# DarianNwankwo/Rollout-Bayesian-Optimization

Measured on AMD Instinct MI355X. Metric: rollout trajectories/sec (MC samples × restarts) at horizon h=3, n=64 GP, higher is better.
Workload: dtype f64

## Files before the change

rollout-bayesian-optimization_amd/csrc/mrbo_rollout.hip:

```cpp
#include <utility>

#include "mrbo_device.h"
#include "bcast_asm.h"
#include "mrbo_lane_tables.h"

#ifndef MRBO_WAVES_PER_SIMD
#define MRBO_WAVES_PER_SIMD 2
#endif
#define MRBO_FNS_CAT_(a, b) a##b
#define MRBO_FNS_CAT(a, b) MRBO_FNS_CAT_(a, b)
#define MRBO_FNS MRBO_FNS_CAT(fmax, MRBO_FMAX)
#ifndef MRBO_WAVES_PER_SIMD_GL
#define MRBO_WAVES_PER_SIMD_GL 1
#endif

namespace mrbo {
inline namespace MRBO_FNS {

constexpr double PAD_FAR = 1e100;

template <int D, int RPL, int HW = 1>
struct Lay {
  static constexpr int D1 = D + 1;
  static constexpr int BS = (D1 + 1) & ~1;
  static constexpr int NR = RPL * WAVE;
  static constexpr int LANES = WAVE / HW;
  static constexpr int NRL = RPL * LANES;
  static constexpr bool SQ = (RPL == 1);
  static constexpr bool BC = (RPL <= 2);
  static constexpr int FR0 = 0;
  static constexpr int BROWS = FR0 + FMAX;
  static constexpr int NG = D1 * (D1 + 1) / 2;
  static constexpr int NH = D * (D + 1) / 2;
  static constexpr int R_VAL = 0;
  static constexpr int R_G = 8;
  static constexpr int NGC = (NG - 1 + 15) / 16;
  static constexpr int R_MF = R_G + 16 * NGC;
  static constexpr int NMF = D * (1 + FMAX);
  static constexpr int NMFC = (NMF + 15) / 16;
  static constexpr int NPAIR = D * D + 2 * D;
  static constexpr int NPC = (NPAIR + 15) / 16;
  static constexpr int NHC = (NH + 1 + 15) / 16;
  static constexpr int REDN_A = R_MF + 16 * NMFC;
  static constexpr int REDN_B = 16 * (NPC > NHC ? NPC : NHC);
  static constexpr int REDN = ((REDN_A > REDN_B ? REDN_A : REDN_B) + 1) & ~1;
  static constexpr int U_X = 0;
  static constexpr int DE = (D + 1) & ~1;
  static constexpr int U_XB = U_X + (DE > 8 ? DE : 8);
  static constexpr int U_XF = U_XB + (DE > 8 ? DE : 8);
  static constexpr int U_YF = U_XF + FMAX * D;
  static constexpr int U_GF = U_YF + FMAX;
  static constexpr int U_DINV = U_GF + FMAX * D;
  static constexpr int U_CF = U_DINV + FMAX * FMAX;
  static constexpr int U_FMIN = U_CF + (FMAX + 1) * FMAX;
  static constexpr int U_SC = U_FMIN + FMAX + 1;
  static constexpr int U_GMU = U_SC + 20;
  static constexpr int U_GSIG = U_GMU + D;
  static constexpr int U_GAL = U_GSIG + D;
  static constexpr int U_MIX = U_GAL + D;
  static constexpr int U_G = U_MIX + D;
  static constexpr int U_H = U_G + D1 * D1;
  static constexpr int U_YFV = U_H + D * D;
  static constexpr int U_WF = U_YFV + FMAX * D1;
  static constexpr int U_PF = U_WF + FMAX;
  static constexpr int U_GMU0 = U_PF + FMAX * D;
  static constexpr int U_XBAR = U_GMU0 + D;
  static constexpr int U_ACC = U_XBAR + FMAX * D;
  static constexpr int U_YBAR = U_ACC + FMAX * D;
  static constexpr int U_DX = U_YBAR + FMAX + 1;
  static constexpr int U_NX = U_DX + D;
  static constexpr int U_NG = U_NX + D;
  static constexpr int U_NP = U_NG + D;
  static constexpr int U_LB = U_NP + D;
  static constexpr int U_UB = U_LB + D;
  static constexpr int U_HF = U_UB + D;
  static constexpr int U_STAMP = U_HF + FMAX * (D + 2);
  static constexpr int U_KC = U_STAMP + NSTAMP_SLOTS;
  static constexpr bool LTAB = (RPL == 1);
  static constexpr int U_TAB = ((U_KC + 15) + 1) & ~1;
  static constexpr int U_SIZE = LTAB ? ((U_TAB + LaneTables<D, FMAX>::DOUBLES + 1) & ~1) : U_TAB;
  static constexpr int G12 = 3 * NRL;
  static constexpr int EC = SQ ? (2 * FMAX + 1) * NRL : 0;
// ... 308 lines not shown
      for (int q = 0; q < 8; ++q) v[q] = fill(16 * ch + q);
      hw_reduce<HW, 8>(v, red + 16 * ch, lane);
    } else {
      double v[16];
#pragma unroll
      for (int q = 0; q < 16; ++q) v[q] = fill(16 * ch + q);
      hw_reduce<HW, 16>(v, red + 16 * ch, lane);
    }
  }
}

template <int K>
__device__ __forceinline__ void gl_bcast_product_k(double (&acc)[K], const double (&v)[K], const double* lb, int nrows) {
#pragma unroll
  for (int p = 0; p < 2; ++p) {
    if (16 * p >= nrows) break;
    double l[4][8];
#pragma unroll
    for (int u = 0; u < 8; ++u) {
      l[0][u] = lb[(16 * p + u) * WAVE];
      l[1][u] = lb[(16 * p + 8 + u) * WAVE];
      l[2][u] = lb[(16 * (p + 2) + u) * WAVE];
      l[3][u] = lb[(16 * (p + 2) + 8 + u) * WAVE];
    }
    double bp[K], bp2[K];
#pragma unroll
    for (int c = 0; c < K; ++c) {
      if (p == 0) row_blocks<0>(v[c], bp[c], bp2[c]);
      else row_blocks<1>(v[c], bp[c], bp2[c]);
    }
    BcastRegAsm<K, 0>::run(acc, bp, l[0]);
    BcastRegAsm<K, 8>::run(acc, bp, l[1]);
    if (16 * (p + 2) < nrows) {
      BcastRegAsm<K, 0>::run(acc, bp2, l[2]);
      BcastRegAsm<K, 8>::run(acc, bp2, l[3]);
    }
  }
}

template <int K>
__device__ __forceinline__ void gl_bcast_product(double (&acc)[K], const double (&v)[K], const double* lb, int nrows) {
  if constexpr (K > 9) {
    gl_bcast_product<8>(head8(acc), head8(v), lb, nrows);
    gl_bcast_product<K - 8>(tail8(acc), tail8(v), lb, nrows);
  } else {
    gl_bcast_product_k<K>(acc, v, lb, nrows);
  }
}

template <int K, int LD, int NLB>
__device__ __forceinline__ void gl_block(double (&acc)[K], const double (&v)[K], const double* Lg, const double* LinvL,
                                         int b, bool fwd, int lane, int nrows) {
  const int li = NLB > 0 ? gl_lds_slot(b) : -1;
  if (li >= 0) {
    const double* sq = LinvL + (long long)li * WAVE * LD;
    if (fwd) bcast_product<K, LD, 1, false>(acc, v, sq + lane, nrows);
    else bcast_product<K, 1, 1, false>(acc, v, sq + lane * LD, nrows);
  } else {
    gl_bcast_product<K>(acc, v, Lg + (long long)b * WAVE * WAVE + lane, nrows);
  }
}

template <int D, int RPL, int HW>
__device__ __forceinline__ bool newton_pg_ok(WaveCtx<D, RPL, HW>& W, const KParams& kp);

struct NewtonState {
  double f, ft, dec, t;
  int it, ls;
  int st;
  bool trial;
  int why;
};
enum { NT_STOP = 0,
       NT_BACKTRACK = 1,
       NT_CONTINUE = 2 };
template <int D, int RPL, int HW>
__device__ __forceinline__ int newton_after_value(WaveCtx<D, RPL, HW>& W, const KParams& kp, int S, NewtonState& ns);

constexpr int EV_RT = -1;

template <int D, int RPL, int HW, int MODE = EV_RT>
__device__ __forceinline__ int evaluate(WaveCtx<D, RPL, HW>& W, const KParams& kp, int S, int mode_rt,
                                        LaneRes<D, RPL, HW>& lr, int kst = 0, bool back_after = false,
                                        NewtonState* nt = nullptr) {
  using Ly = Lay<D, RPL, HW>;
  constexpr int D1 = Ly::D1, BS = Ly::BS, NR = Ly::NR;
  constexpr bool FUSABLE = Ly::SQ && HW == 1;
  static_assert(MODE == EV_RT || (MODE >= EV_VALUE && MODE <= EV_GSTART), "evaluate: MODE");
  const int mode = MODE == EV_RT ? mode_rt : MODE;
  int lane = W.lane;
  asm volatile("" : "+v"(lane));
  const int nf = S + 1;
  double* U = W.U;
  double* B = W.B;
  double* red = W.red;
  const unsigned* tab = reinterpret_cast<const unsigned*>(U + Ly::U_TAB);
  const bool all_cols = (mode != EV_VALUE);
  const bool do_val = (mode != EV_GRADC);
  STAMP(W, 8);

  double x[D];
#pragma unroll
  for (int a = 0; a < D; ++a) x[a] = U[Ly::U_X + a];

  double Ev[RPL][FMAX];
#pragma unroll
  for (int s = 0; s < RPL; ++s) {
    lr.cb[s] = W.C[(long long)(S + 1) * Ly::NRL + lane + WAVE * s];
#pragma unroll
    for (int r = 0; r < FMAX; ++r) Ev[s][r] = W.E[(long long)r * Ly::NRL + lane + WAVE * s];
#pragma unroll
    for (int r = 0; r < FMAX; ++r) Ev[s][r] = (r < nf) ? Ev[s][r] : 0.0;
  }

  const int N = W.N;
  double acc[RPL][D1];
  if (mode != EV_BACK) {
  double Bown[RPL][D1];
  double rf[D], psif = 0.0, g1f = 0.0, g2f = 0.0;
  const bool rows_kept = (mode == EV_GRADC);
#pragma unroll
  for (int s = 0; s < RPL; ++s) {
    double r[D], rho2 = 0.0;
#pragma unroll
    for (int a = 0; a < D; ++a) { r[a] = x[a] - W.X0[s][a]; rho2 = fma(r[a], r[a], rho2); }
    if (rows_kept) {
      const double g1 = W.G12[3 * (lane + WAVE * s)];
      const bool v = W.rowv(kp, s);
      Bown[s][0] = 0.0;
#pragma unroll
      for (int a = 0; a < D; ++a) Bown[s][1 + a] = v ? g1 * r[a] : 0.0;
      continue;
    }
    double psi, g1, g2;
    if constexpr (RPL == 1) {
      const int fl = lane < nf ? lane : 0;
      double rho2f = 0.0;
#pragma unroll
      for (int a = 0; a < D; ++a) { rf[a] = x[a] - U[Ly::U_XF + fl * D + a]; rho2f = fma(rf[a], rf[a], rho2f); }
      rad_eval2<MODE != EV_RT>(W.rad, rho2, rho2f, psi, g1, g2, psif, g1f, g2f);
    } else {
      rad_eval(W.rad, rho2, psi, g1, g2);
    }
    const bool v = W.rowv(kp, s);
    Bown[s][0] = v ? psi : 0.0;
#pragma unroll
    for (int a = 0; a < D; ++a) Bown[s][1 + a] = v ? g1 * r[a] : 0.0;
    W.G12[3 * (lane + WAVE * s)] = g1;
    W.G12[3 * (lane + WAVE * s) + 1] = g2;
  }
  if (lane < nf && !rows_kept) {
    double r[D], psi, g1, g2;
    if constexpr (RPL == 1) {
#pragma unroll
      for (int a = 0; a < D; ++a) r[a] = rf[a];
      psi = psif;
      g1 = g1f;
      g2 = g2f;
    } else {
      double rho2 = 0.0;
#pragma unroll
      for (int a = 0; a < D; ++a) { r[a] = x[a] - U[Ly::U_XF + lane * D + a]; rho2 = fma(r[a], r[a], rho2); }
      rad_eval(W.rad, rho2, psi, g1, g2);
    }
    double* row = B + (Ly::FR0 + lane) * BS;
    row[0] = psi;
#pragma unroll
    for (int a = 0; a < D; ++a) row[1 + a] = g1 * r[a];
    {
      double* hf = U + Ly::U_HF + lane * (D + 2);
#pragma unroll
      for (int a = 0; a < D; ++a) hf[a] = r[a];
      hf[D] = g1;
      hf[D + 1] = g2;
    }
  }
  wave_sync();
  STAMP(W, 0);

#pragma unroll
  for (int s = 0; s < RPL; ++s)
#pragma unroll
    for (int c = 0; c < D1; ++c) acc[s][c] = 0.0;
  if constexpr (Ly::BC) {
    auto nrows = [&](int t) { const int n = N - WAVE * t; return n < WAVE ? n : WAVE; };
    const bool fold = Ly::SQ && HW == 1 && N > 48;
#ifdef MRBO_BC_DIAG_FOLD
    constexpr bool DFOLD = !Ly::SQ && HW == 1;
#else
    constexpr bool DFOLD = false;
#endif
    if (mode == EV_VALUE) {
#pragma unroll
      for (int s = 0; s < RPL; ++s) {
        double a1[1] = {0.0};
#pragma unroll
        for (int t = 0; t <= s; ++t) {
          const double v1[1] = {Bown[t][0]};
          if (fold) bcast_fold_fwd<1>(a1, v1, W.Linv, lane);
          else if (DFOLD && s == t && nrows(t) > 48) bcast_fold_fwd<1>(a1, v1, W.Linv + Ly::blk(s, t) * Ly::BLK, lane);
          else bcast_product<1, Ly::LD, HW>(a1, v1, W.Linv + Ly::blk(s, t) * Ly::BLK + lane, nrows(t));
        }
        acc[s][0] = a1[0];
      }
    } else if (mode == EV_GSTART) {
      if constexpr (Ly::SQ) acc[0][0] = W.YTAB[(long long)kst * NR + lane];
    } else if (mode == EV_GRADC) {
#pragma unroll
      for (int s = 0; s < RPL; ++s) {
        double ag[D];
#pragma unroll
        for (int a = 0; a < D; ++a) ag[a] = 0.0;
#pragma unroll
        for (int t = 0; t <= s; ++t) {
          double vg[D];
#pragma unroll
          for (int a = 0; a < D; ++a) vg[a] = Bown[t][1 + a];
          if (fold) bcast_fold_fwd<D>(ag, vg, W.Linv, lane);
          else if (DFOLD && s == t && nrows(t) > 48) bcast_fold_fwd<D>(ag, vg, W.Linv + Ly::blk(s, t) * Ly::BLK, lane);
          else bcast_product<D, Ly::LD, HW>(ag, vg, W.Linv + Ly::blk(s, t) * Ly::BLK + lane, nrows(t));
        }
#pragma unroll
        for (int a = 0; a < D; ++a) acc[s][1 + a] = ag[a];
        acc[s][0] = W.G12[3 * (lane + WAVE * s) + 2];
      }
    } else {
#pragma unroll
      for (int s = 0; s < RPL; ++s)
#pragma unroll
        for (int t = 0; t <= s; ++t) {
          if (fold) bcast_fold_fwd<D1>(acc[s], Bown[t], W.Linv, lane);
          else if (DFOLD && s == t && nrows(t) > 48) bcast_fold_fwd<D1>(acc[s], Bown[t], W.Linv + Ly::blk(s, t) * Ly::BLK, lane);
          else bcast_product<D1, Ly::LD, HW>(acc[s], Bown[t], W.Linv + Ly::blk(s, t) * Ly::BLK + lane, nrows(t));
        }
    }
  } else {
    auto nrows = [&](int t) { const int n = N - WAVE * t; return n < WAVE ? n : WAVE; };
    const double* L0 = W.Linv + lane;
    if (mode == EV_VALUE) {
#pragma unroll
      for (int s = 0; s < RPL; ++s) {
        double a1[1] = {0.0};
#pragma unroll
        for (int t = 0; t <= s; ++t) {
          const double v1[1] = {Bown[t][0]};
          gl_block<1, Ly::LD, Ly::NLB>(a1, v1, W.Linv, W.LinvL, Ly::blk(s, t), true, lane, nrows(t));
        }
        acc[s][0] = a1[0];
      }
    } else if (mode == EV_GRADC) {
#pragma unroll
      for (int s = 0; s < RPL; ++s) {
// ... 94 lines not shown
#pragma unroll
    for (int r = 0; r < FMAX; ++r) {
      if (r < nf) {
        g00_v = fma(yf[r], yf[r], g00_v);
        mu_v = fma(U[Ly::U_CF + (S + 1) * FMAX + r], bf[r], mu_v);
      }
    }
    if (lane < FMAX) {
      double mine = 0.0;
#pragma unroll
      for (int r = 0; r < FMAX; ++r) mine = (lane == r) ? yf[r] : mine;
      if (lane < nf) U[Ly::U_YFV + lane * D1] = mine;
    }
    if (lane == 0) {
      U[Ly::U_G] = g00_v;
      U[Ly::U_SC + SC_MU] = mu_v;
    }
  }
  if (all_cols) {
  {
    const int ncol = D;
    for (int t = lane; t < (FMAX * D <= Ly::LANES ? Ly::LANES : FMAX * D); t += Ly::LANES) {
      if (t >= nf * ncol) break;
      int r = t / ncol, c = 1 + t % ncol;
      if constexpr (Ly::LTAB) {
        const unsigned tw = tab[t];
        r = lane_field(tw, LaneWord::R, LaneWord::W3);
        c = lane_field(tw, LaneWord::C, LaneWord::W5);
      }
      double y = red[Ly::R_MF + D + r * D + (c - 1)];
      for (int q = 0; q <= r; ++q) y = fma(U[Ly::U_DINV + r * FMAX + q], B[(Ly::FR0 + q) * BS + c], y);
      U[Ly::U_YFV + r * D1 + c] = y;
      if constexpr (FMAX * D <= Ly::LANES) break;
    }
  }
  wave_sync();
  {
    auto gram_entry = [&](int t) {
      int a = 0, b;
      if constexpr (Ly::LTAB) {
        const unsigned tw = tab[t];
        a = lane_field(tw, LaneWord::GA, LaneWord::W5);
        b = lane_field(tw, LaneWord::GB, LaneWord::W5);
      } else {
        int rem = t;
#pragma unroll
        for (int aa = 0; aa < D1; ++aa) if (a == aa && rem >= D1 - aa) { rem -= D1 - aa; a = aa + 1; }
        b = a + rem;
      }
      double g = (mode == EV_GSTART) ? W.GTAB[kst * Ly::NG + t] : red[Ly::R_G + t - 1];
      for (int r = 0; r < nf; ++r) g = fma(U[Ly::U_YFV + r * D1 + a], U[Ly::U_YFV + r * D1 + b], g);
      U[Ly::U_G + a * D1 + b] = g;
      U[Ly::U_G + b * D1 + a] = g;
    };
    auto gmu_entry = [&](int c) {
      double mu = red[Ly::R_MF + c - 1];
      for (int r = 0; r < nf; ++r) mu = fma(U[Ly::U_CF + (S + 1) * FMAX + r], B[(Ly::FR0 + r) * BS + c], mu);
      U[Ly::U_GMU + c - 1] = mu;
    };
    if constexpr (HW == 2) {
      static_assert(Ly::NG <= 16 && 16 + D <= 32, "half-wave Gram placement");
      if (lane > 0 && lane < Ly::NG) gram_entry(lane);
      if (lane >= 16 && lane < 16 + D) gmu_entry(lane - 15);
    } else if constexpr (Ly::NG <= 49) {
      if (lane > 0 && lane < Ly::NG) gram_entry(lane);
      if (lane >= 49 && lane < 48 + D1) gmu_entry(lane - 48);
    } else {
      for (int t = lane; t < Ly::NG; t += WAVE)
        if (t > 0) gram_entry(t);
      if (lane >= 1 && lane <= D) gmu_entry(lane);
    }
  }
  wave_sync();
  }
  STAMP(W, 3);

  double isig_f;
  EIp e_f;
  if (do_val) {
  const double mu = mu_v;
  const double var = KCV(PSI0) - g00_v;
  double sig, isig;
  sig_isig(var, sig, isig);
  const double fmin = U[Ly::U_FMIN + S + 1];
  const EIp e = rule_partials(kp.rule, mu, sig, KCV(THETA), fmin, KCV(SIGTOL), isig);
  double alpha = e.g;
  if (kp.cost) {
    double gc[D];
    const double c = cost_eval<D>(kp, x, gc);
    double gmax = 0.0;
#pragma unroll
    for (int a = 0; a < D; ++a) gmax = fmax(gmax, fabs(gc[a]));
    alpha = e.g / c;
    if (lane == 0) {
      U[Ly::U_SC + SC_ARAW] = e.g;
      U[Ly::U_SC + SC_COSTC] = c;
      U[Ly::U_SC + SC_GCMAX] = gmax;
    }
  }
  if (lane == 0) {
    U[Ly::U_SC + SC_SIG] = sig;
    U[Ly::U_SC + SC_ISIG] = isig;
    U[Ly::U_SC + SC_VAR] = var;
    U[Ly::U_SC + SC_ALPHA] = alpha;
    U[Ly::U_SC + SC_GMU] = e.gmu;
    U[Ly::U_SC + SC_GSIG] = e.gsig;
    U[Ly::U_SC + SC_GMUMU] = e.gmumu;
    U[Ly::U_SC + SC_GSIGSIG] = e.gsigsig;
    U[Ly::U_SC + SC_GMUTH] = e.gmuth;
    U[Ly::U_SC + SC_GSIGTH] = e.gsigth;
    U[Ly::U_SC + SC_FMIN] = fmin;
  }
  if (mode == EV_VALUE) {
    wave_sync();
    STAMP(W, 4);
    if constexpr (FUSABLE) {
      if (nt != nullptr) {
        nt->why = newton_after_value<D, RPL, HW>(W, kp, S, *nt);
        if (nt->why != NT_CONTINUE || !kp.newton_fused) return 0;
        if constexpr (MODE != EV_GRADC)
          return EVR_GRAD | evaluate<D, RPL, HW, EV_GRADC>(W, kp, S, EV_GRADC, lr, kst, true);
      }
    }
    return 0;
  }
  isig_f = isig;
  e_f = e;
  } else {
    isig_f = U[Ly::U_SC + SC_ISIG];
    e_f.gmu = U[Ly::U_SC + SC_GMU];
    e_f.gsig = U[Ly::U_SC + SC_GSIG];
    e_f.gmuth = U[Ly::U_SC + SC_GMUTH];
    e_f.gsigth = U[Ly::U_SC + SC_GSIGTH];
  }
  if (lane < D) {
    const double gs = -U[Ly::U_G + (1 + lane) * D1] * isig_f;
    const double gm = U[Ly::U_GMU + lane];
    U[Ly::U_GSIG + lane] = gs;
    double gal = e_f.gmu * gm + e_f.gsig * gs;
    double mix = gm * e_f.gmuth + gs * e_f.gsigth;
    if (kp.cost) {
      double gc[D];
      (void)cost_eval<D>(kp, x, gc);
      const double gca = lane_pick<D>(gc, lane);
      const double c = U[Ly::U_SC + SC_COSTC], araw = U[Ly::U_SC + SC_ARAW];
      gal = gal / c - (araw / (c * c)) * gca;
      mix = mix / c - rule_gth(kp.rule, e_f.gmu, U[Ly::U_SC + SC_SIG]) * gca / (c * c);
    }
    U[Ly::U_GAL + lane] = gal;
    U[Ly::U_MIX + lane] = mix;
  }
  if (mode == EV_GRAD || mode == EV_GRADC || mode == EV_GSTART) {
    wave_sync();
    STAMP(W, 4);
    if (!back_after) return 0;
    if (lane < D) U[Ly::U_NG + lane] = -U[Ly::U_GAL + lane];
    wave_sync();
    if (!newton_pg_ok<D, RPL, HW>(W, kp)) return 0;
    STAMP(W, 12);
  }
  } else {
#pragma unroll
    for (int s = 0; s < RPL; ++s) acc[s][0] = W.G12[3 * (lane + WAVE * s) + 2];
  }
  wave_sync();
  EIp e;
  e.gmu = U[Ly::U_SC + SC_GMU];
  e.gsig = U[Ly::U_SC + SC_GSIG];
  e.gmumu = U[Ly::U_SC + SC_GMUMU];
  e.gsigsig = U[Ly::U_SC + SC_GSIGSIG];

  STAMP(W, 4);
  const bool rich = (mode == EV_RICH);
  {
    double wv[RPL], pv[RPL][D];
#pragma unroll
    for (int s = 0; s < RPL; ++s) {
      wv[s] = 0.0;
#pragma unroll
      for (int a = 0; a < D; ++a) pv[s][a] = 0.0;
    }
    if constexpr (Ly::BC) {
      auto nrows = [&](int t) { const int n = N - WAVE * t; return n < WAVE ? n : WAVE; };
      const bool fold = Ly::SQ && HW == 1 && N > 48;
#ifdef MRBO_BC_DIAG_FOLD
      constexpr bool DFOLD = !Ly::SQ && HW == 1;
#else
      constexpr bool DFOLD = false;
#endif
#pragma unroll
      for (int s = 0; s < RPL; ++s) {
        if (rich) {
          double a7[D1];
#pragma unroll
          for (int c = 0; c < D1; ++c) a7[c] = 0.0;
#pragma unroll
          for (int t = s; t < RPL; ++t) {
            if (fold) bcast_fold_bwd<D1>(a7, acc[t], W.Linv, lane);
            else if (DFOLD && s == t && nrows(t) > 48) bcast_fold_bwd<D1>(a7, acc[t], W.Linv + Ly::blk(t, s) * Ly::BLK, lane);
            else bcast_product<D1, 1, HW>(a7, acc[t], W.Linv + Ly::blk(t, s) * Ly::BLK + lane * Ly::LD, nrows(t));
          }
          wv[s] = a7[0];
#pragma unroll
          for (int a = 0; a < D; ++a) pv[s][a] = a7[1 + a];
        } else {
          double a1[1] = {0.0};
#pragma unroll
          for (int t = s; t < RPL; ++t) {
            const double v1[1] = {acc[t][0]};
            if (fold) bcast_fold_bwd<1>(a1, v1, W.Linv, lane);
            else if (DFOLD && s == t && nrows(t) > 48) bcast_fold_bwd<1>(a1, v1, W.Linv + Ly::blk(t, s) * Ly::BLK, lane);
            else bcast_product<1, 1, HW>(a1, v1, W.Linv + Ly::blk(t, s) * Ly::BLK + lane * Ly::LD, nrows(t));
          }
          wv[s] = a1[0];
        }
      }
    } else {
      auto nrows = [&](int t) { const int n = N - WAVE * t; return n < WAVE ? n : WAVE; };
      const double* LT = W.LinvT + lane;
#pragma unroll
      for (int s = 0; s < RPL; ++s) {
        if (rich) {
          double a7[D1];
#pragma unroll
          for (int c = 0; c < D1; ++c) a7[c] = 0.0;
#pragma unroll
          for (int t = s; t < RPL; ++t)
            gl_block<D1, Ly::LD, Ly::NLB>(a7, acc[t], W.LinvT, W.LinvL, Ly::blk(t, s), false, lane, nrows(t));
          wv[s] = a7[0];
#pragma unroll
          for (int a = 0; a < D; ++a) pv[s][a] = a7[1 + a];
        } else {
          double a1[1] = {0.0};
#pragma unroll
          for (int t = s; t < RPL; ++t) {
            const double v1[1] = {acc[t][0]};
            gl_block<1, Ly::LD, Ly::NLB>(a1, v1, W.LinvT, W.LinvL, Ly::blk(t, s), false, lane, nrows(t));
          }
          wv[s] = a1[0];
        }
      }
    }
#pragma unroll
    for (int s = 0; s < RPL; ++s) {
#pragma unroll
      for (int r = 0; r < FMAX; ++r) {
        if (r >= nf) break;
        const double er = Ev[s][r];
// ... 32 lines not shown
    for (int s = 0; s < RPL; ++s) {
#pragma unroll
      for (int a = 0; a < D; ++a) nv[s][a] = x[a] - W.X0[s][a];
      const double coef = W.rowv(kp, s) ? (e.gmu * lr.cb[s] - gsig_over * lr.w[s]) : 0.0;
      ca[s] = coef * W.G12[3 * (lane + WAVE * s) + 1];
      tb[s] = coef * W.G12[3 * (lane + WAVE * s)];
    }
    wave_sync();
    auto hval = [&](int t) {
      double s_ = 0.0;
      if (t < Ly::NH) {
        int a = 0, rem = t;
#pragma unroll
        for (int aa = 0; aa < D; ++aa) if (a == aa && rem >= D - aa) { rem -= D - aa; a = aa + 1; }
        const int b = a + rem;
#pragma unroll
        for (int s = 0; s < RPL; ++s) s_ = fma(ca[s], nv[s][a] * nv[s][b], s_);
      } else if (t == Ly::NH) {
#pragma unroll
        for (int s = 0; s < RPL; ++s) s_ += tb[s];
      }
      return s_;
    };
    constexpr int HTAIL = (Ly::NH + 1) % 16;
    constexpr int HFULL = (HTAIL > 0 && HTAIL <= 8) ? (Ly::NH + 1) / 16 : Ly::NHC;
#pragma unroll
    for (int ch = 0; ch < HFULL; ++ch) {
      double vv[16];
#pragma unroll
      for (int q = 0; q < 16; ++q) vv[q] = hval(16 * ch + q);
      hw_reduce<HW, 16>(vv, red + 16 * ch, lane);
    }
    if constexpr (HFULL < Ly::NHC) {
      double vv[8];
#pragma unroll
      for (int q = 0; q < 8; ++q) vv[q] = hval(16 * HFULL + q);
      hw_reduce<HW, 8>(vv, red + 16 * HFULL, lane);
    }
  }
  wave_sync();
  STAMP(W, 6);
  for (int he = lane; he < (Ly::NH <= Ly::LANES ? Ly::LANES : Ly::NH); he += Ly::LANES) {
    if (he >= Ly::NH) break;
    int a = 0, b;
    if constexpr (Ly::LTAB) {
      const unsigned tw = tab[he];
      a = lane_field(tw, LaneWord::HA, LaneWord::W5);
      b = lane_field(tw, LaneWord::HB, LaneWord::W5);
    } else {
      int rem = he;
#pragma unroll
      for (int aa = 0; aa < D; ++aa) if (a == aa && rem >= D - aa) { rem -= D - aa; a = aa + 1; }
      b = a + rem;
    }
    const double gma = U[Ly::U_GMU + a], gmb = U[Ly::U_GMU + b];
    const double gsa = U[Ly::U_GSIG + a], gsb = U[Ly::U_GSIG + b];
    const double rdiag = red[Ly::NH];
    double hv = red[he] + ((a == b) ? rdiag : 0.0);
    for (int r = 0; r < nf; ++r) {
      const double* hf = U + Ly::U_HF + r * (D + 2);
      const double coef = e.gmu * U[Ly::U_CF + (S + 1) * FMAX + r] - gsig_over * U[Ly::U_WF + r];
      hv = fma(coef * hf[D + 1], hf[a] * hf[b], hv);
      if (a == b) hv = fma(coef, hf[D], hv);
    }
    hv += e.gmumu * gma * gmb + e.gsigsig * gsa * gsb - gsig_over * (gsa * gsb + U[Ly::U_G + (1 + a) * D1 + 1 + b]);
    if (kp.cost) {
      double gc[D];
      (void)cost_eval<D>(kp, x, gc);
      const double gca = lane_pick<D>(gc, a), gcb = lane_pick<D>(gc, b);
      const double c = U[Ly::U_SC + SC_COSTC], araw = U[Ly::U_SC + SC_ARAW];
      hv = (hv - U[Ly::U_GAL + a] * gcb - gca * U[Ly::U_GAL + b]) / c - (araw / (c * c)) * cost_hess<D>(kp, c, a, b);
    }
    U[Ly::U_H + a * D + b] = hv;
    U[Ly::U_H + b * D + a] = hv;
    if constexpr (Ly::NH <= Ly::LANES) break;
  }
  wave_sync();
  STAMP(W, 7);
  return EVR_BACK;
}

template <int D, int RPL, int HW>
__device__ __forceinline__ int condition(WaveCtx<D, RPL, HW>& W, const KParams& kp, int S, double yv, const double* gy,
                         const LaneRes<D, RPL, HW>& lr) {
  using Ly = Lay<D, RPL, HW>;
  constexpr int NR = Ly::NR;
  double* U = W.U;
  const int lane = W.ln();
  const int nf = S + 1;
  const double g00 = U[Ly::U_G];
  const double mu = U[Ly::U_SC + SC_MU];
  const double l22sq = KCV(PSI0) + KCV(SN2) - g00;
  if (!(l22sq > 0.0)) return 4;
  const double inv = 1.0 / sqrt(l22sq);
  const double gam = (yv - mu) / l22sq;
#pragma unroll
  for (int s = 0; s < RPL; ++s) {
    const int i = lane + WAVE * s;
    W.E[(long long)nf * Ly::NRL + i] = W.rowv(kp, s) ? -lr.w[s] * inv : 0.0;
    W.C[(long long)(S + 2) * Ly::NRL + i] = W.rowv(kp, s) ? (lr.cb[s] - gam * lr.w[s]) : 0.0;
  }
  wave_sync();
  if (lane < nf) {
    const double wq = U[Ly::U_WF + lane];
    U[Ly::U_DINV + nf * FMAX + lane] = -wq * inv;
    U[Ly::U_CF + (S + 2) * FMAX + lane] = U[Ly::U_CF + (S + 1) * FMAX + lane] - gam * wq;
  }
  if (lane == nf) {
    U[Ly::U_DINV + nf * FMAX + nf] = inv;
    U[Ly::U_CF + (S + 2) * FMAX + nf] = gam;
    U[Ly::U_YF + nf] = yv;
    const double fm = U[Ly::U_FMIN + S + 1];
    U[Ly::U_FMIN + S + 2] = (yv < fm) ? yv : fm;
  }
  double gmine = 0.0;
#pragma unroll
  for (int a = 0; a < D; ++a) gmine = (a == lane) ? gy[a] : gmine;
  if (lane < D) {
    U[Ly::U_XF + nf * D + lane] = U[Ly::U_X + lane];
    U[Ly::U_GF + nf * D + lane] = gmine;
  }
  wave_sync();
  return 0;
}

template <int D, int RPL, int HW>
__device__ __forceinline__ int draw_factor(WaveCtx<D, RPL, HW>& W, double (&Lc)[Lay<D, RPL, HW>::NG]) {
  using Ly = Lay<D, RPL, HW>;
  constexpr int D1 = Ly::D1;
  const double* U = W.U;
#define TRI(i, j) ((i) * ((i) + 1) / 2 + (j))
#pragma unroll
  for (int j = 0; j < D1; ++j) {
    const double kjj = (j == 0) ? KCV(PSI0) : -KCV(D2PSI0);
    double sdiag = kjj - U[Ly::U_G + j * D1 + j];
#pragma unroll
    for (int k = 0; k < j; ++k) sdiag -= Lc[TRI(j, k)] * Lc[TRI(j, k)];
    if (!(sdiag > 0.0)) return 2;
    double ljj, ij;
    sqrt_rsqrt(sdiag, ljj, ij);
    Lc[TRI(j, j)] = ljj;
#pragma unroll
    for (int i = j + 1; i < D1; ++i) {
      double t = -U[Ly::U_G + j * D1 + i];
#pragma unroll
      for (int k = 0; k < j; ++k) t -= Lc[TRI(i, k)] * Lc[TRI(j, k)];
      Lc[TRI(i, j)] = t * ij;
    }
  }
#undef TRI
  return 0;
}

template <int D, int RPL, int HW>
__device__ __forceinline__ int draw(WaveCtx<D, RPL, HW>& W, const KParams& kp, const double* z, double& yv, double* gy,
                                    const double* hdr = nullptr) {
  using Ly = Lay<D, RPL, HW>;
  constexpr int D1 = Ly::D1;
  const double* U = W.U;
  double Lc[Ly::NG];
#define TRI(i, j) ((i) * ((i) + 1) / 2 + (j))
  if (hdr) {
    if (hdr[RT_FAIL] != 0.0) return 2;
#pragma unroll
    for (int i = 0; i < Ly::NG; ++i) Lc[i] = hdr[RT_GMU + 2 * D + i];
  } else if (draw_factor<D, RPL, HW>(W, Lc)) {
    return 2;
  }
  double out[D1];
  out[0] = U[Ly::U_SC + SC_MU];
#pragma unroll
  for (int a = 0; a < D; ++a) out[1 + a] = U[Ly::U_GMU + a];
#pragma unroll
  for (int a = 0; a < D1; ++a) {
    double s = 0.0;
#pragma unroll
    for (int k = 0; k <= a; ++k) s += Lc[TRI(a, k)] * z[k];
    out[a] += s;
  }
#undef TRI
  yv = out[0];
#pragma unroll
  for (int a = 0; a < D; ++a) gy[a] = out[1 + a];
  return 0;
}

template <int D>
__device__ __forceinline__ bool chol_packed(double (&A)[D * (D + 1) / 2], double (&idg)[D]) {
#define TRI(i, j) ((i) * ((i) + 1) / 2 + (j))
  bool ok = true;
#pragma unroll
  for (int j = 0; j < D; ++j) {
    double s = A[TRI(j, j)];
#pragma unroll
    for (int k = 0; k < j; ++k) s -= A[TRI(j, k)] * A[TRI(j, k)];
    ok = ok && (s > 0.0);
    if (!ok) return false;
    double ljj;
    sqrt_rsqrt(s, ljj, idg[j]);
    A[TRI(j, j)] = ljj;
#pragma unroll
    for (int i = j + 1; i < D; ++i) {
      double t = A[TRI(i, j)];
#pragma unroll
      for (int k = 0; k < j; ++k) t -= A[TRI(i, k)] * A[TRI(j, k)];
      A[TRI(i, j)] = t * idg[j];
    }
  }
#undef TRI
  return ok;
}

template <int D, int RPL, int HW>
__device__ __forceinline__ bool newton_pg_ok(WaveCtx<D, RPL, HW>& W, const KParams& kp) {
  using Ly = Lay<D, RPL, HW>;
  const double* U = W.U;
  const int lane = W.ln();
  const int a = lane < D ? lane : 0;
  const double xs = U[Ly::U_NX + a], gs = U[Ly::U_NG + a], lb = U[Ly::U_LB + a], ub = U[Ly::U_UB + a];
  const bool act = ((xs <= lb) & (gs > 0.0)) | ((xs >= ub) & (gs < 0.0));
  const bool fr = (lane < D) & !act;
  const unsigned long long fm = hw_ballot<HW>(fr, W.half);
  const unsigned long long big = hw_ballot<HW>(fr & (fabs(gs) > KCV(GTOL)), W.half);
  if (lane == 0) W.U[Ly::U_SC + SC_FREE] = (double)(unsigned)fm;
  return big != 0ull;
}

template <int D, int RPL, int HW, bool ALL_FREE>
__device__ __forceinline__ bool newton_direction_fm(WaveCtx<D, RPL, HW>& W, const KParams& kp, int fm) {
  using Ly = Lay<D, RPL, HW>;
  constexpr int NH = D * (D + 1) / 2;
  double* U = W.U;
  const int lane = W.ln();
  bool fr[D];
  double gs[D];
#pragma unroll
  for (int a = 0; a < D; ++a) {
    fr[a] = ALL_FREE || ((fm >> a) & 1);
    gs[a] = U[Ly::U_NG + a];
  }
  double A0[NH];
#pragma unroll
  for (int i = 0; i < D; ++i)
#pragma unroll
    for (int j = 0; j <= i; ++j) {
      const double h = U[Ly::U_H + i * D + j];
      A0[i * (i + 1) / 2 + j] = (fr[i] && fr[j]) ? -h : ((i == j) ? 1.0 : 0.0);
    }
  double tau = 0.0, hmax = 0.0;
#pragma unroll
  for (int i = 0; i < D; ++i) {
    double off = 0.0;
#pragma unroll
// ... 322 lines not shown
  for (int q = threadIdx.x; q < NR * ns; q += blockDim.x) {
    const int i = q / ns, k = q - (q / ns) * ns;
    double v = 0.0;
    if (i < kp.N) {
      double rho2 = 0.0;
#pragma unroll
      for (int a = 0; a < D; ++a) {
        const double r = clampd(xs[k * D + a], kp.lbs[a], kp.ubs[a]) - kp.X0[(long long)a * NR + i];
        rho2 = fma(r, r, rho2);
      }
      double g1, g2;
      rad_eval(rad, rho2, v, g1, g2);
    }
    kxb[q] = v;
  }
  __syncthreads();
  const int lane = threadIdx.x & (WAVE - 1), wv = threadIdx.x / WAVE, nw = blockDim.x / WAVE;
  double* red = smem + tb.end + (long long)wv * Ly::WAVE_LDS;
  double* ytab = kp.ytab;
  for (int k = wv; k < ns; k += nw) {
    double bv[Ly::D1], acc[Ly::D1];
    double rho2 = 0.0, r[D];
#pragma unroll
    for (int a = 0; a < D; ++a) {
      r[a] = clampd(xs[k * D + a], kp.lbs[a], kp.ubs[a]) - kp.X0[(long long)a * NR + lane];
      rho2 = fma(r[a], r[a], rho2);
    }
    double psi, g1, g2;
    rad_eval(rad, rho2, psi, g1, g2);
    const bool v = lane < kp.N;
    bv[0] = v ? psi : 0.0;
#pragma unroll
    for (int a = 0; a < D; ++a) bv[1 + a] = v ? g1 * r[a] : 0.0;
#pragma unroll
    for (int c = 0; c < Ly::D1; ++c) acc[c] = 0.0;
    bcast_product<Ly::D1, Ly::LD>(acc, bv, smem + lane, kp.N);
    if (store_y) ytab[(long long)k * NR + lane] = acc[0];
#pragma unroll
    for (int ch = 0; ch < (Ly::NG + 15) / 16; ++ch) {
      double gv[16];
#pragma unroll
      for (int q = 0; q < 16; ++q) {
        const int t = 16 * ch + q;
        double s_ = 0.0;
        if (t < Ly::NG) {
          int a = 0, rem = t;
#pragma unroll
          for (int aa = 0; aa < Ly::D1; ++aa) if (a == aa && rem >= Ly::D1 - aa) { rem -= Ly::D1 - aa; a = aa + 1; }
          s_ = acc[a] * acc[a + rem];
        }
        gv[q] = s_;
      }
      wave_reduce<16>(gv, red + 16 * ch, lane);
    }
    wave_sync();
    for (int t = lane; t < Ly::NG; t += WAVE) smem[tb.gtab + (long long)k * Ly::NG + t] = red[t];
    wave_sync();
  }
  __syncthreads();
}

template <int D, int RPL, int HW>
__device__ __forceinline__ void batch_start_values(WaveCtx<D, RPL, HW>& W, const KParams& kp, int S, double& f_lane,
                                                   double& gm_lane, double& gs_lane, double& sig_lane,
                                                   double& a_lane, unsigned long long& stopmask,
                                                   unsigned long long& xnanmask, bool& varneg) {
  using Ly = Lay<D, RPL, HW>;
  constexpr int NR = Ly::NR;
  const double* U = W.U;
  const int lane = W.ln();
  const int ns = kp.nstarts, nf = S + 1;
  const bool split = HW == 1 && ns <= 32;
  const int kl = split ? (lane & 31) : lane;
  const int hf = split ? (lane >> 5) : 0;
  const bool act = lane < ns;
  const int k = kl < ns ? kl : 0;
  double x[D];
#pragma unroll
  for (int a = 0; a < D; ++a) x[a] = clampd(W.XS[k * D + a], U[Ly::U_LB + a], U[Ly::U_UB + a]);
  double amu = 0.0, ae[FMAX];
#pragma unroll
  for (int r = 0; r < FMAX; ++r) ae[r] = 0.0;
  const double* cS = W.C + (long long)(S + 1) * Ly::NRL;
  if constexpr (!Ly::SQ) {
    double cv[RPL], ev[RPL][FMAX];
#pragma unroll
    for (int s2 = 0; s2 < RPL; ++s2) {
      const int i = lane + WAVE * s2;
      cv[s2] = cS[i];
#pragma unroll
      for (int r = 0; r < FMAX; ++r) ev[s2][r] = W.E[(long long)r * Ly::NRL + i];
    }
    double* sums = W.SUMS;
    auto load_pair = [&](int kc, double (&kxp)[2][RPL]) {
#pragma unroll
      for (int kk = 0; kk < 2; ++kk) {
        const int kq = (kc + kk < ns) ? kc + kk : (kc < ns ? kc : 0);
#pragma unroll
        for (int s2 = 0; s2 < RPL; ++s2) kxp[kk][s2] = W.KXB[(long long)kq * NR + lane + WAVE * s2];
      }
    };
    double kxn[2][RPL];
    load_pair(0, kxn);
    for (int kc = 0; kc < ns; kc += 2) {
      double kxc[2][RPL];
#pragma unroll
      for (int kk = 0; kk < 2; ++kk)
#pragma unroll
        for (int s2 = 0; s2 < RPL; ++s2) kxc[kk][s2] = kxn[kk][s2];
      load_pair(kc + 2, kxn);
      double v[16];
#pragma unroll
      for (int kk = 0; kk < 2; ++kk) {
        const double* kx = kxc[kk];
        double a0 = 0.0;
#pragma unroll
        for (int s2 = 0; s2 < RPL; ++s2) a0 = fma(cv[s2], kx[s2], a0);
        v[8 * kk] = a0;
#pragma unroll
        for (int r = 0; r < FMAX; ++r) {
          double a = 0.0;
#pragma unroll
          for (int s2 = 0; s2 < RPL; ++s2) a = fma(ev[s2][r], kx[s2], a);
          v[8 * kk + 1 + r] = a;
        }
        v[8 * kk + 7] = 0.0;
      }
      wave_reduce<16>(v, sums + 8 * kc, lane);
    }
    wave_sync();
    amu = sums[8 * k];
#pragma unroll
    for (int r = 0; r < FMAX; ++r) ae[r] = sums[8 * k + 1 + r];
    wave_sync();
  } else if (split) {
#pragma unroll 8
    for (int j = 0; j < NR / 2; ++j) {
      const int i = 2 * j + hf;
      const double kv = W.KXB[i * ns + k];
      amu = fma(cS[i], kv, amu);
#pragma unroll
      for (int r = 0; r < FMAX; ++r) ae[r] = fma(W.E[(long long)r * Ly::NRL + i], kv, ae[r]);
    }
    amu = swap_fold<32>(amu, amu);
#pragma unroll
    for (int r = 0; r < FMAX; ++r) ae[r] = swap_fold<32>(ae[r], ae[r]);
  } else {
#pragma unroll 8
    for (int i = 0; i < W.N; ++i) {
      const double kv = W.KXB[i * ns + k];
      amu = fma(cS[i], kv, amu);
#pragma unroll
      for (int r = 0; r < FMAX; ++r) ae[r] = fma(W.E[(long long)r * Ly::NRL + i], kv, ae[r]);
    }
  }
  double pf[FMAX];
  if (split) {
#pragma unroll
    for (int e = 0; e < FMAX / 2; ++e) {
      const int q = 2 * e + hf;
      double v = 0.0;
      if (2 * e < nf) {
        double rho2 = 0.0;
#pragma unroll
        for (int a = 0; a < D; ++a) { const double r = x[a] - U[Ly::U_XF + q * D + a]; rho2 = fma(r, r, rho2); }
        double g1, g2;
        rad_eval(W.rad, rho2, v, g1, g2);
      }
      self_swap<32, false>(v, pf[2 * e], pf[2 * e + 1]);
    }
#pragma unroll
    for (int q = 0; q < FMAX; ++q) pf[q] = (q < nf) ? pf[q] : 0.0;
  } else {
#pragma unroll
    for (int q = 0; q < FMAX; ++q) {
      pf[q] = 0.0;
      if (q < nf) {
        double rho2 = 0.0;
#pragma unroll
        for (int a = 0; a < D; ++a) { const double r = x[a] - U[Ly::U_XF + q * D + a]; rho2 = fma(r, r, rho2); }
        double g1, g2;
        rad_eval(W.rad, rho2, pf[q], g1, g2);
      }
    }
  }
  double g00 = W.GTAB[k * Ly::NG], mu = amu;
#pragma unroll
  for (int r = 0; r < FMAX; ++r) {
    if (r < nf) {
      double y = ae[r];
#pragma unroll
      for (int q = 0; q <= r; ++q) y = fma(U[Ly::U_DINV + r * FMAX + q], pf[q], y);
      g00 = fma(y, y, g00);
      mu = fma(U[Ly::U_CF + (S + 1) * FMAX + r], pf[r], mu);
    }
  }
  const double var = KCV(PSI0) - g00;
  double sig, isig;
  sig_isig(var, sig, isig);
  const EIp e = rule_partials(kp.rule, mu, sig, KCV(THETA), U[Ly::U_FMIN + S + 1], KCV(SIGTOL), isig);
  double fval = e.g, cval = 1.0, gcm = 0.0;
  if (kp.cost) {
    double gc[D];
    cval = cost_eval<D>(kp, x, gc);
#pragma unroll
    for (int a = 0; a < D; ++a) gcm = fmax(gcm, fabs(gc[a]));
    fval = e.g / cval;
  }
  bool cert = (e.gmu == 0.0 && e.gsig == 0.0) && (!kp.cost || e.g == 0.0);
  if (!cert && kp.gcert_sig > 0.0) {
    double b = fabs(e.gmu) * KCV(GCMU) * U[Ly::U_SC + SC_CABS] + fabs(e.gsig) * KCV(GCSIG) * isig;
    if (kp.cost) b = b * (1.0 / cval) + fabs(e.g) * gcm / (cval * cval);
    cert = b <= 0.25 * KCV(GTOL);
  }
  f_lane = -fval;
  a_lane = e.g;
  gm_lane = e.gmu;
  gs_lane = e.gsig;
  sig_lane = sig;
  const bool stop = cert || (f_lane != f_lane) || kp.max_iters <= 0;
  bool xn = false;
#pragma unroll
  for (int a = 0; a < D; ++a) xn = xn || (x[a] != x[a]);
  stopmask = hw_ballot<HW>(act && stop, W.half);
  xnanmask = hw_ballot<HW>(act && xn, W.half);
  varneg = hw_ballot<HW>(act && var < 0.0, W.half) != 0;
}

template <int D, int RPL, int HW>
__device__ __forceinline__ int multistart(WaveCtx<D, RPL, HW>& W, const KParams& kp, int S, Counters& nevals,
                                          LaneRes<D, RPL, HW>& lr, int k0, int k1) {
  using Ly = Lay<D, RPL, HW>;
  double* U = W.U;
  const int lane = W.ln();
  int st = 0;
  int best = -1;
// ... 287 lines not shown
template <int D, int RPL, int HW>
__device__ __forceinline__ void restart_row_load(WaveCtx<D, RPL, HW>& W, const KParams& kp, int r, LaneRes<D, RPL, HW>& lr) {
  using Ly = Lay<D, RPL, HW>;
  static_assert(RPL == 1 && HW == 1, "restart table: square full-wave layout");
  static_assert(rtab_header(D) <= Ly::REDN, "restart-table header staged in the reduction area");
  double* U = W.U;
  double* red = W.red;
  const int lane = W.ln();
  const double* row = kp.rtab + (long long)r * rtab_stride(D, Ly::NR);
  lr.w[0] = row[lane];
  lr.cb[0] = W.C[lane];
#pragma unroll
  for (int a = 0; a < D; ++a) lr.P[0][a] = 0.0;
  for (int q = lane; q < rtab_header(D); q += WAVE) red[q] = row[Ly::NR + q];
  wave_sync();
  if (lane == 0) {
    U[Ly::U_SC + SC_VAR] = red[RT_VAR];
    U[Ly::U_SC + SC_MU] = red[RT_MU];
    U[Ly::U_G] = red[RT_G00];
    U[Ly::U_SC + SC_SIG] = red[RT_SIG];
  }
  if (lane < D) {
    U[Ly::U_GMU + lane] = red[RT_GMU + lane];
    U[Ly::U_GSIG + lane] = red[RT_GMU + D + lane];
  }
  wave_sync();
}

template <int D, int RPL, int HW>
__device__ __forceinline__ void trajectory(WaveCtx<D, RPL, HW>& W, const KParams& kp, long long tr) {
  using Ly = Lay<D, RPL, HW>;
  constexpr int D1 = Ly::D1, NR = Ly::NR;
  double* U = W.U;
  const int lane = W.ln();
  const int M = kp.M, h = kp.h;
  const int r = (int)(tr / M), m = (int)(tr % M);
  Counters nevals;
  int st = 0;
  LaneRes<D, RPL, HW> lr;

#pragma unroll
  for (int s = 0; s < RPL; ++s) W.C[lane + WAVE * s] = kp.c0[lane + WAVE * s];
  if (lane == 0) U[Ly::U_FMIN] = U[Ly::U_KC + KC_FMINB];
  const bool bsolve = kp.base_solve != 0;
  if (lane < D) {
    if (!bsolve) U[Ly::U_X + lane] = kp.x0s[(long long)r * D + lane];
    U[Ly::U_LB + lane] = kp.lbs[lane];
    U[Ly::U_UB + lane] = kp.ubs[lane];
  }
  wave_sync();

  const int kend = bsolve ? 1 : h;
  for (int k = bsolve ? 1 : 0; k <= kend; ++k) {
    const int S = bsolve ? -1 : k - 1;
    if (k > 0) {
      if (kp.replay && !bsolve) {
        if (lane < D) U[Ly::U_X + lane] = kp.replay[(long long)lane + D * ((k - 1) + (long long)h * (m + (long long)M * r))];
        wave_sync();
      } else {
        st |= multistart<D, RPL, HW>(W, kp, S, nevals, lr, bsolve ? (int)tr : 0, bsolve ? (int)tr + 1 : kp.nstarts);
        if (bsolve) {
          if (lane == 0) kp.status[tr] = st & ~8;
          if (kp.evals && lane == 0) {
            kp.evals[NCOUNT * tr + 0] = nevals.grad;
            kp.evals[NCOUNT * tr + 1] = nevals.value;
            kp.evals[NCOUNT * tr + 2] = nevals.hess;
            kp.evals[NCOUNT * tr + 3] = 0;
            kp.evals[NCOUNT * tr + 4] = 0;
          }
          wave_sync();
          return;
        }
        if (st) break;
        if (lane < D) U[Ly::U_X + lane] = U[Ly::U_XB + lane];
        wave_sync();
      }
    }
    if (kp.policy && lane < D) kp.policy[(long long)lane + D * (k + (long long)(h + 1) * (m + (long long)M * r))] = U[Ly::U_X + lane];
    bool tabled = false;
    if constexpr (Ly::SQ && HW == 1) {
      tabled = (k == 0) && kp.rtab != nullptr;
      if (tabled) restart_row_load<D, RPL, HW>(W, kp, r, lr);
    }
    if (!tabled) evaluate<D, RPL, HW>(W, kp, S, EV_DRAW, lr);
    if (U[Ly::U_SC + SC_VAR] < 0.0) { st |= 1; break; }
    if (k == 0 && lane < D) U[Ly::U_GMU0 + lane] = U[Ly::U_GMU + lane];
    double yv, gy[D];
    if (kp.ghq_w) {
      const long long ik = (long long)m + (long long)M * k;
      const double tk = kp.ghq_nodes[ik], wk = kp.ghq_w[ik];
      yv = U[Ly::U_SC + SC_MU] + 1.4142135623730951 * U[Ly::U_SC + SC_SIG] * tk;
#pragma unroll
      for (int a = 0; a < D; ++a) gy[a] = wk * (U[Ly::U_GMU + a] + 1.4142135623730951 * U[Ly::U_GSIG + a] * tk);
    } else {
      double z[D1];
#pragma unroll
      for (int a = 0; a < D1; ++a) z[a] = kp.rn[(long long)m + (long long)M * a + (long long)M * D1 * k];
      st |= draw<D, RPL, HW>(W, kp, z, yv, gy, tabled ? W.red : nullptr);
      if (st) break;
    }
    wave_sync();
    st |= condition<D, RPL, HW>(W, kp, S, yv, gy, lr);
    STAMP(W, 10);
    if (st) break;
  }
  wave_sync();
  const long long oidx = (long long)m + (long long)M * r;
  if (kp.obs && lane <= h) kp.obs[oidx * (h + 1) + lane] = st ? qnan() : U[Ly::U_YF + lane];
  if (kp.evals && lane == 0) {
    kp.evals[NCOUNT * oidx + 0] = nevals.grad;
    kp.evals[NCOUNT * oidx + 1] = nevals.value;
    kp.evals[NCOUNT * oidx + 2] = nevals.hess;
    kp.evals[NCOUNT * oidx + 3] = 0;
    kp.evals[NCOUNT * oidx + 4] = 0;
  }
  if (st) {
    if (lane == 0) { kp.values[oidx] = qnan(); kp.status[oidx] = st; if (kp.grad_theta) kp.grad_theta[oidx] = qnan(); }
    if (kp.grad_x && lane < D) kp.grad_x[oidx * D + lane] = qnan();
    return;
  }
  STAMP(W, 11);
  double bo = U[Ly::U_YF];
  int t = 0;
  for (int k = 1; k <= h; ++k) { const double yk = U[Ly::U_YF + k]; if (yk < bo) { bo = yk; t = k; } }
  double value = fmax(kp.fmini - bo, 0.0);
  if (kp.ghq_w) value *= kp.ghq_w[(long long)m + (long long)M * t] * 0.5641895835477563;
  double gth = 0.0;
  bool grad_zero = true;
  if (kp.with_gradient && kp.fmini > bo) {
    if (t == 0) {
      grad_zero = false;
      if (lane < D) U[Ly::U_ACC + lane] = U[Ly::U_GF + lane];
      if (lane == 0) U[Ly::U_YBAR] = 0.0;
      if (lane < D) U[Ly::U_GMU0 + lane] = 0.0;
      wave_sync();
    } else {
      grad_zero = false;
      for (int q = lane; q < FMAX * D; q += Ly::LANES) { U[Ly::U_ACC + q] = 0.0; U[Ly::U_XBAR + q] = 0.0; }
      if (lane <= FMAX) U[Ly::U_YBAR + lane] = 0.0;
      wave_sync();
      if (lane == 0) U[Ly::U_YBAR + t] = 1.0;
      wave_sync();
      for (int j = t; j >= 1; --j) {
        wave_sync();
        if (lane < D) {
          U[Ly::U_DX + lane] = kp.dual_y
              ? kp.dual_y[(long long)lane + D * ((j - 1) + (long long)h * (m + (long long)M * r))]
              : dual_uniform_k(__builtin_bit_cast(unsigned long long, U[Ly::U_KC + KC_DXKEY]),
                               (long long)(kp.sample_offset + m), j, lane);
        }
        wave_sync();
        for (int i = j; i <= t; ++i) {
          if (i > j) {
            bool xz = true;
#pragma unroll
            for (int a = 0; a < D; ++a) xz = xz && (U[Ly::U_XBAR + (i - 1) * D + a] == 0.0);
            if (xz) continue;
          }
          rich_eval_at<D, RPL, HW>(W, kp, i, lr);
          ++nevals.rich;
          if (i == j) {
            double Hm[D][D], xd[D], det;
#pragma unroll
            for (int a = 0; a < D; ++a)
#pragma unroll
              for (int b = 0; b < D; ++b) Hm[a][b] = U[Ly::U_H + b * D + a];
            const double ybj = U[Ly::U_YBAR + j];
#pragma unroll
            for (int a = 0; a < D; ++a) xd[a] = -U[Ly::U_GF + (j - 1) * D + a] * ybj - U[Ly::U_ACC + j * D + a];
            const bool nonsing = lu_det_solve<D>(Hm, xd, det, true);
            bool zero = !(det >= KCV(HTOL));
            if (det != det) zero = false;
            if (zero) {
#pragma unroll
              for (int a = 0; a < D; ++a) xd[a] = 0.0;
            } else if (!nonsing) {
              st |= 16;
            }
            double gq = 0.0;
            double mine = 0.0;
#pragma unroll
            for (int a = 0; a < D; ++a) { gq = fma(U[Ly::U_MIX + a], xd[a], gq); if (a == lane) mine = xd[a]; }
            gth += gq;
            wave_sync();
            if (lane < D) U[Ly::U_XBAR + (j - 1) * D + lane] = mine;
// ... 398 lines not shown
```

Baseline: 7.993 million.

## Skip unused gradient work at final rollout step and specialize start-value row loops

At the last horizon step, the draw evaluation skips EI partials, gradient-of-alpha, hessian-feature stores and the backward part of the evaluation, because only the sampled y value is needed. Conditioning at that step skips the Cholesky/factor update and only records y, x and the first gradient. The start-value row loop is also specialized by the number of fantasized points, so the inner loop over FMAX rows runs only nf iterations. This risks correctness if later code reads state such as U_GAL, U_HF or the factor update after the final step.

New measurement: 8.074 million (median of 6 runs). +1.0%, better.

```diff
diff --git a/rollout-bayesian-optimization_amd/csrc/mrbo_rollout.hip b/rollout-bayesian-optimization_amd/csrc/mrbo_rollout.hip
--- a/rollout-bayesian-optimization_amd/csrc/mrbo_rollout.hip
+++ b/rollout-bayesian-optimization_amd/csrc/mrbo_rollout.hip
@@ -1,3 +1,4 @@
+#include <type_traits>
 #include <utility>
 
 #include "mrbo_device.h"
@@ -472,7 +473,7 @@
 template <int D, int RPL, int HW, int MODE = EV_RT>
 __device__ __forceinline__ int evaluate(WaveCtx<D, RPL, HW>& W, const KParams& kp, int S, int mode_rt,
                                         LaneRes<D, RPL, HW>& lr, int kst = 0, bool back_after = false,
-                                        NewtonState* nt = nullptr) {
+                                        NewtonState* nt = nullptr, bool draw_back = true) {
   using Ly = Lay<D, RPL, HW>;
   constexpr int D1 = Ly::D1, BS = Ly::BS, NR = Ly::NR;
   constexpr bool FUSABLE = Ly::SQ && HW == 1;
@@ -487,6 +488,7 @@
   const unsigned* tab = reinterpret_cast<const unsigned*>(U + Ly::U_TAB);
   const bool all_cols = (mode != EV_VALUE);
   const bool do_val = (mode != EV_GRADC);
+  const bool keep = (mode != EV_DRAW) || !Ly::BC;
   STAMP(W, 8);
 
   double x[D];
@@ -557,7 +559,7 @@
     row[0] = psi;
 #pragma unroll
     for (int a = 0; a < D; ++a) row[1 + a] = g1 * r[a];
-    {
+    if (keep) {
       double* hf = U + Ly::U_HF + lane * (D + 2);
 #pragma unroll
       for (int a = 0; a < D; ++a) hf[a] = r[a];
@@ -818,6 +820,14 @@
   const double var = KCV(PSI0) - g00_v;
   double sig, isig;
   sig_isig(var, sig, isig);
+  isig_f = isig;
+  if (!keep) {
+    if (lane == 0) {
+      U[Ly::U_SC + SC_SIG] = sig;
+      U[Ly::U_SC + SC_ISIG] = isig;
+      U[Ly::U_SC + SC_VAR] = var;
+    }
+  } else {
   const double fmin = U[Ly::U_FMIN + S + 1];
   const EIp e = rule_partials(kp.rule, mu, sig, KCV(THETA), fmin, KCV(SIGTOL), isig);
   double alpha = e.g;
@@ -860,8 +870,8 @@
     }
     return 0;
   }
-  isig_f = isig;
   e_f = e;
+  }
   } else {
     isig_f = U[Ly::U_SC + SC_ISIG];
     e_f.gmu = U[Ly::U_SC + SC_GMU];
@@ -873,6 +883,7 @@
     const double gs = -U[Ly::U_G + (1 + lane) * D1] * isig_f;
     const double gm = U[Ly::U_GMU + lane];
     U[Ly::U_GSIG + lane] = gs;
+    if (keep) {
     double gal = e_f.gmu * gm + e_f.gsig * gs;
     double mix = gm * e_f.gmuth + gs * e_f.gsigth;
     if (kp.cost) {
@@ -885,6 +896,7 @@
     }
     U[Ly::U_GAL + lane] = gal;
     U[Ly::U_MIX + lane] = mix;
+    }
   }
   if (mode == EV_GRAD || mode == EV_GRADC || mode == EV_GSTART) {
     wave_sync();
@@ -900,6 +912,7 @@
     for (int s = 0; s < RPL; ++s) acc[s][0] = W.G12[3 * (lane + WAVE * s) + 2];
   }
   wave_sync();
+  if (mode == EV_DRAW && !draw_back) { STAMP(W, 4); STAMP(W, 5); return 0; }
   EIp e;
   e.gmu = U[Ly::U_SC + SC_GMU];
   e.gsig = U[Ly::U_SC + SC_GSIG];
@@ -1098,7 +1111,7 @@
 
 template <int D, int RPL, int HW>
 __device__ __forceinline__ int condition(WaveCtx<D, RPL, HW>& W, const KParams& kp, int S, double yv, const double* gy,
-                         const LaneRes<D, RPL, HW>& lr) {
+                         const LaneRes<D, RPL, HW>& lr, bool last = false) {
   using Ly = Lay<D, RPL, HW>;
   constexpr int NR = Ly::NR;
   double* U = W.U;
@@ -1108,6 +1121,18 @@
   const double mu = U[Ly::U_SC + SC_MU];
   const double l22sq = KCV(PSI0) + KCV(SN2) - g00;
   if (!(l22sq > 0.0)) return 4;
+  if (last) {
+    if (lane == nf) U[Ly::U_YF + nf] = yv;
+    if (lane < D) U[Ly::U_XF + nf * D + lane] = U[Ly::U_X + lane];
+    if (nf == 0) {
+      double g0 = 0.0;
+#pragma unroll
+      for (int a = 0; a < D; ++a) g0 = (a == lane) ? gy[a] : g0;
+      if (lane < D) U[Ly::U_GF + lane] = g0;
+    }
+    wave_sync();
+    return 0;
+  }
   const double inv = 1.0 / sqrt(l22sq);
   const double gam = (yv - mu) / l22sq;
 #pragma unroll
@@ -1170,7 +1195,7 @@
 
 template <int D, int RPL, int HW>
 __device__ __forceinline__ int draw(WaveCtx<D, RPL, HW>& W, const KParams& kp, const double* z, double& yv, double* gy,
-                                    const double* hdr = nullptr) {
+                                    const double* hdr = nullptr, bool y_only = false) {
   using Ly = Lay<D, RPL, HW>;
   constexpr int D1 = Ly::D1;
   const double* U = W.U;
@@ -1185,6 +1210,13 @@
   }
   double out[D1];
   out[0] = U[Ly::U_SC + SC_MU];
+  if (y_only) {
+    double s = 0.0;
+    s += Lc[0] * z[0];
+    out[0] += s;
+    yv = out[0];
+    return 0;
+  }
 #pragma unroll
   for (int a = 0; a < D; ++a) out[1 + a] = U[Ly::U_GMU + a];
 #pragma unroll
@@ -1673,6 +1705,30 @@
 #pragma unroll
   for (int r = 0; r < FMAX; ++r) ae[r] = 0.0;
   const double* cS = W.C + (long long)(S + 1) * Ly::NRL;
+  auto sq_rows = [&](auto nfc) {
+    constexpr int NF = decltype(nfc)::value;
+    if (split) {
+#pragma unroll 8
+      for (int j = 0; j < NR / 2; ++j) {
+        const int i = 2 * j + hf;
+        const double kv = W.KXB[i * ns + k];
+        amu = fma(cS[i], kv, amu);
+#pragma unroll
+        for (int r = 0; r < NF; ++r) ae[r] = fma(W.E[(long long)r * Ly::NRL + i], kv, ae[r]);
+      }
+      amu = swap_fold<32>(amu, amu);
+#pragma unroll
+      for (int r = 0; r < NF; ++r) ae[r] = swap_fold<32>(ae[r], ae[r]);
+    } else {
+#pragma unroll 8
+      for (int i = 0; i < W.N; ++i) {
+        const double kv = W.KXB[i * ns + k];
+        amu = fma(cS[i], kv, amu);
+#pragma unroll
+        for (int r = 0; r < NF; ++r) ae[r] = fma(W.E[(long long)r * Ly::NRL + i], kv, ae[r]);
+      }
+    }
+  };
   if constexpr (!Ly::SQ) {
     double cv[RPL], ev[RPL][FMAX];
 #pragma unroll
@@ -1724,25 +1780,21 @@
 #pragma unroll
     for (int r = 0; r < FMAX; ++r) ae[r] = sums[8 * k + 1 + r];
     wave_sync();
-  } else if (split) {
-#pragma unroll 8
-    for (int j = 0; j < NR / 2; ++j) {
-      const int i = 2 * j + hf;
-      const double kv = W.KXB[i * ns + k];
-      amu = fma(cS[i], kv, amu);
-#pragma unroll
-      for (int r = 0; r < FMAX; ++r) ae[r] = fma(W.E[(long long)r * Ly::NRL + i], kv, ae[r]);
-    }
-    amu = swap_fold<32>(amu, amu);
-#pragma unroll
-    for (int r = 0; r < FMAX; ++r) ae[r] = swap_fold<32>(ae[r], ae[r]);
   } else {
-#pragma unroll 8
-    for (int i = 0; i < W.N; ++i) {
-      const double kv = W.KXB[i * ns + k];
-      amu = fma(cS[i], kv, amu);
-#pragma unroll
-      for (int r = 0; r < FMAX; ++r) ae[r] = fma(W.E[(long long)r * Ly::NRL + i], kv, ae[r]);
+    static_assert(FMAX == 4 || FMAX == 6, "batch_start_values: one row-loop copy per nf");
+    switch (nf) {
+      case 0: sq_rows(std::integral_constant<int, 0>{}); break;
+      case 1: sq_rows(std::integral_constant<int, 1>{}); break;
+      case 2: sq_rows(std::integral_constant<int, 2>{}); break;
+      case 3: sq_rows(std::integral_constant<int, 3>{}); break;
+      default:
+        if constexpr (FMAX == 4) {
+          sq_rows(std::integral_constant<int, 4>{});
+        } else {
+          if (nf == 4) sq_rows(std::integral_constant<int, 4>{});
+          else if (nf == 5) sq_rows(std::integral_constant<int, 5>{});
+          else sq_rows(std::integral_constant<int, 6>{});
+        }
     }
   }
   double pf[FMAX];
@@ -2196,7 +2248,8 @@
       tabled = (k == 0) && kp.rtab != nullptr;
       if (tabled) restart_row_load<D, RPL, HW>(W, kp, r, lr);
     }
-    if (!tabled) evaluate<D, RPL, HW>(W, kp, S, EV_DRAW, lr);
+    const bool last = Ly::BC && (k == h), y_only = last && k > 0;
+    if (!tabled) evaluate<D, RPL, HW>(W, kp, S, EV_DRAW, lr, 0, false, nullptr, !last);
     if (U[Ly::U_SC + SC_VAR] < 0.0) { st |= 1; break; }
     if (k == 0 && lane < D) U[Ly::U_GMU0 + lane] = U[Ly::U_GMU + lane];
     double yv, gy[D];
@@ -2204,17 +2257,19 @@
       const long long ik = (long long)m + (long long)M * k;
       const double tk = kp.ghq_nodes[ik], wk = kp.ghq_w[ik];
       yv = U[Ly::U_SC + SC_MU] + 1.4142135623730951 * U[Ly::U_SC + SC_SIG] * tk;
-#pragma unroll
-      for (int a = 0; a < D; ++a) gy[a] = wk * (U[Ly::U_GMU + a] + 1.4142135623730951 * U[Ly::U_GSIG + a] * tk);
+      if (!y_only) {
+#pragma unroll
+        for (int a = 0; a < D; ++a) gy[a] = wk * (U[Ly::U_GMU + a] + 1.4142135623730951 * U[Ly::U_GSIG + a] * tk);
+      }
     } else {
       double z[D1];
 #pragma unroll
       for (int a = 0; a < D1; ++a) z[a] = kp.rn[(long long)m + (long long)M * a + (long long)M * D1 * k];
-      st |= draw<D, RPL, HW>(W, kp, z, yv, gy, tabled ? W.red : nullptr);
+      st |= draw<D, RPL, HW>(W, kp, z, yv, gy, tabled ? W.red : nullptr, y_only);
       if (st) break;
     }
     wave_sync();
-    st |= condition<D, RPL, HW>(W, kp, S, yv, gy, lr);
+    st |= condition<D, RPL, HW>(W, kp, S, yv, gy, lr, last);
     STAMP(W, 10);
     if (st) break;
   }
```
